# m-dayani/EORB_SLAM

Measured on AMD Instinct MI355X. Metric: front-end frames/s (event-accumulate + extract + match) per GPU; HBM GB/s vs roofline, higher is better.
Workload: dtype f32; 1 GPU; BASELINE.json configs[1]: synthetic 1000000 events/slice on 240x180 (shapes generator, DAVIS sensor pixels; raw (x,y,t,p) records resolved on the GPU through the calibrator's undistortion maps built from the EvETHZ intrinsics, as the reference loader does on the CPU), ev2im_gauss sigma=1 -> ORB-1000 (1.2, 4 levels, FAST 10/0, edge 19) -> SearchForInitialization vs previous slice; input=raw, sequences_per_gpu=1, parallelism=1 GPU

## Files before the change

### eorb_slam_amd/csrc/ev_slots.hip

```cpp
#include "eorb_ctx.h"
#include "ev_common.h"
#include "dev_math.h"
#include "sl_hot_asm.h"
#include <algorithm>
#include <memory>
#include <stdlib.h>
#include <string.h>
#include <vector>

namespace eorb {

constexpr uint32_t kNoSlot = 0xffu;
typedef uint16_t slot_entry;
constexpr uint32_t kEntryTag = 0x1000u;
constexpr int kSlotScatWaves = 8;
constexpr uint16_t kNoGeo = 0xffffu;
constexpr int kCountWaves = 16;

__global__ void sl_assign_kernel(const uint32_t* __restrict__ src_info, int nsrc, int W, int H, int h, int TX,
                                 uint32_t* __restrict__ tile_nslots, uint2* __restrict__ slot_tab, uint16_t* __restrict__ slot_geo,
                                 int* __restrict__ info)
{
    const int i = blockIdx.x * blockDim.x + threadIdx.x;
    if (i >= nsrc) { if (i == nsrc) slot_geo[i] = kNoGeo; return; }
    const uint32_t w = src_info[i];
    const int xi = (int)(int16_t)(w & 0xffff), yi = (int)(int16_t)(w >> 16);
    uint2 o = make_uint2(0u, 0xffffffffu);
    if (xi != -32768) {
        const int x0 = max(xi - h, 0), x1 = min(xi + h, W - 1), y0 = max(yi - h, 0), y1 = min(yi + h, H - 1);
        if (x1 >= x0 && y1 >= y0) {
            const int tx0 = x0 >> 3, tx1 = x1 >> 3, ty0 = y0 >> 3, ty1 = y1 >> 3;
            const int nx = tx1 - tx0 + 1, ny = ty1 - ty0 + 1;
            uint32_t slots = 0xffffffffu;
            for (int dy = 0; dy < ny; dy++)
                for (int dx = 0; dx < nx; dx++) {
                    uint32_t s = atomicAdd(&tile_nslots[(ty0 + dy) * TX + tx0 + dx], 1u);
                    if (s >= kNoSlot) { atomicOr(&info[2], 1); s = 0; }
                    const int sh = 8 * (dy * 2 + dx);
                    slots = (slots & ~(0xffu << sh)) | (s << sh);
                }
            o.x = (uint32_t)tx0 | ((uint32_t)ty0 << 8) | ((uint32_t)nx << 16) | ((uint32_t)ny << 18);
            o.y = slots;
        }
    }
    slot_tab[i] = o;
    slot_geo[i] = o.x ? (uint16_t)((o.x & 0x7f) | (((o.x >> 8) & 0x7f) << 7) | ((((o.x >> 16) & 3) - 1) << 14) | ((((o.x >> 18) & 3) - 1) << 15)) : kNoGeo;
}

__global__ __launch_bounds__(1024) void sl_rowbase_kernel(const uint32_t* __restrict__ nslots, int NT, uint32_t* __restrict__ rowbase,
                                                          int* __restrict__ info)
{
    __shared__ uint32_t wsum[16];
    __shared__ uint32_t wmax[16];
    const int tid = threadIdx.x, lane = tid & 63, wave = tid >> 6;
    const int per = (NT + 1023) / 1024;
    const int t0 = tid * per, t1 = min(t0 + per, NT);
    uint32_t mine = 0, mx = 0;
    for (int t = t0; t < t1; t++) { const uint32_t v = nslots[t]; mine += v; mx = max(mx, v); }
    uint32_t incl = (uint32_t)wave_incl_scan((int)mine);
#pragma unroll
    for (int d = 32; d >= 1; d >>= 1) mx = max(mx, (uint32_t)__shfl_xor((int)mx, d, 64));
    if (lane == 63) wsum[wave] = incl;
    if (lane == 0) wmax[wave] = mx;
    __syncthreads();
    uint32_t before = incl - mine;
    for (int w = 0; w < wave; w++) before += wsum[w];
    for (int t = t0; t < t1; t++) { rowbase[t] = before; before += nslots[t]; }
    if (tid == 1023) {
        uint32_t m = 0;
        for (int w = 0; w < 16; w++) m = max(m, wmax[w]);
// ... 366 lines not shown
        if (tid == NTHR - 1) loff[NT] = (uint16_t)before;
    }
    __syncthreads();
    const uint64_t lt_mask = (lane == 0) ? 0ull : (~0ull >> (64 - lane));
    uint16_t* cw = cntw + wave * NTp;
    const int txr = (TX + R - 1) / R;
    int mbits = 1; while ((1 << mbits) < txr * ((TY + R - 1) / R)) mbits++;
#pragma unroll
    for (int s = 0; s < SMAX; s++) {
        if (s >= S) break;
        const uint32_t rg = rng[s];
        const int tx0 = rg & 0xff, ty0 = (rg >> 8) & 0xff, tx1 = tx0 + (int)((rg >> 16) & 3) - 1, ty1 = ty0 + (int)((rg >> 18) & 3) - 1;
        const bool valid = rg != 0u;
        const uint16_t kloc = (uint16_t)(wave * Q + s * 64 + lane);
#pragma unroll
        for (int cy = 0; cy < R; cy++) {
#pragma unroll
            for (int cx = 0; cx < R; cx++) {
                const int tx = tx0 + ((cx - tx0 % R) + R) % R;
                const int ty = ty0 + ((cy - ty0 % R) + R) % R;
                const bool has = valid && tx <= tx1 && ty <= ty1;
                uint64_t m = __ballot(has);
                if (m == 0ull) continue;
                const int key = has ? ty * TX + tx : 0;
                const int mkey = has ? (ty / R) * txr + (tx / R) : 0;
                for (int b = 0; b < mbits; b++) {
                    const bool bit = (mkey >> b) & 1;
                    const uint64_t bal = __ballot(bit);
                    m &= bit ? bal : ~bal;
                }
                if (has) {
                    const int rank = __popcll(m & lt_mask);
                    const uint32_t base = cw[key];
                    sidx[(uint32_t)loff[key] + base + rank] = (uint16_t)(kloc | ((tx - tx0) << 11) | ((ty - ty0) << 13));
                    if (rank == 0) cw[key] = (uint16_t)(base + (uint32_t)__popcll(m));
                }
            }
        }
    }
    __syncthreads();
    slot_entry* out = entries + (size_t)slice_ebase[cd.slice];
    const int E = loff[NT];
    for (int p = tid; p < E; p += NTHR) {
        const uint32_t sv = sidx[p];
        const int k = sv & 0x7ff;
        const int dx = (sv >> 11) & 3, dy = (sv >> 13) & 3;
        const uint32_t r0 = prng[k];
        const int t = ((int)(r0 >> 8) + dy) * TX + (int)(r0 & 0xff) + dx;
        const uint32_t slot = (pay[k] >> (8 * (dy * 2 + dx))) & 0xffu;
        out[(size_t)gbase[t] + (uint32_t)(p - (int)loff[t])] = (slot_entry)(kEntryTag | slot);
    }
}

template <int stride, int NW >
__global__ __launch_bounds__(64 * NW) void sl_scatter_rank_kernel(const eorb_raw_event* __restrict__ ev, const ChunkDesc* __restrict__ chunks,
                                                                              const uint2* __restrict__ slot_tab, int LW, int LH, int TX, int NT,
                                                                              int chunk_cap, const int64_t* __restrict__ slice_ebase,
                                                                              const uint32_t* __restrict__ segbase, const uint32_t* __restrict__ tile_base,
                                                                              slot_entry* __restrict__ entries)
{
    extern __shared__ unsigned char sm2[];
    __shared__ uint32_t s_wsum[NW];
    constexpr int NTHR = 64 * NW;
    const int tid = threadIdx.x, lane = tid & 63, wave = tid >> 6;
    const int chunk = blockIdx.x;
    const ChunkDesc cd = chunks[chunk];
    const int NTp = (NT + 1) & ~1;
    uint32_t* gbase = (uint32_t*)sm2;
    uint16_t* stile = (uint16_t*)(gbase + NT);
    uint16_t* cntw = stile + (size_t)chunk_cap * 4;
    uint16_t* loff = cntw + NW * NTp;
    uint8_t* sorted = (uint8_t*)(loff + NTp + 2);
    for (int i = tid; i < NW * NTp / 2; i += NTHR) ((uint32_t*)cntw)[i] = 0u;
    const unsigned char* e = (const unsigned char*)ev + (size_t)cd.start * (size_t)(stride < 0 ? -stride : stride);
    const uint32_t xmask = stride == 4 ? 0x7fffu : 0xffffu;
    const bool hashed = stride < 0 || stride == 2;
    const int Q = (((cd.n + NW - 1) / NW) + 63) & ~63;
    const int S = Q >> 6;
    constexpr int SMAX = 4;
    __syncthreads();
    uint32_t* cw32 = (uint32_t*)(cntw + wave * NTp);
    uint32_t rsrc[SMAX];
#pragma unroll
    for (int s = 0; s < SMAX; s++) {
        const int k = wave * Q + s * 64 + lane;
        const uint32_t q = (s < S && k < cd.n) ? sl_load_rec<stride>(e, k) : 0xffffffffu;
        const int x = q == 0xffffffffu ? 0xffff : (int)(q & xmask), y = (int)(q >> 16);
        if (hashed) { const uint32_t row = q & 0x7fffffffu; rsrc[s] = (row != 0x7fffffffu && row < (uint32_t)LW * (uint32_t)LH) ? row : 0xffffffffu; }
        else rsrc[s] = (x < LW && y < LH) ? (uint32_t)y * (uint32_t)LW + x : 0xffffffffu;
    }
    uint2 rst[SMAX];
#pragma unroll
    for (int s = 0; s < SMAX; s++) rst[s] = rsrc[s] != 0xffffffffu ? slot_tab[rsrc[s]] : make_uint2(0u, 0xffffffffu);
    uint32_t rk[SMAX];
#pragma unroll
    for (int s = 0; s < SMAX; s++) {
        const uint32_t rg = rst[s].x;
        const int nx = (rg >> 16) & 3, ny = (rg >> 18) & 3;
        const int tx0 = rg & 0xff, ty0 = (rg >> 8) & 0xff;
        rk[s] = 0u;
#pragma unroll
        for (int j = 0; j < 4; j++) {
#ifdef EORB_TEST_RANK_ORDER_BUG
            const int dx = j & 1, dy = j >> 1;
#else
            const int dx = ((j & 1) - tx0) & 1, dy = ((j >> 1) - ty0) & 1;
#endif
            if (nx && ny && dx < nx && dy < ny) {
                const int t = (ty0 + dy) * TX + tx0 + dx;
                const uint32_t o = atomicAdd(&cw32[t >> 1], 1u << (16 * (t & 1)));
                rk[s] |= ((o >> (16 * (t & 1))) & 0xffu) << (8 * j);
            }
        }
    }
    __syncthreads();
#if defined(EORB_KO_SCAT) && EORB_KO_SCAT == 1
    if (rk[0] == 0x12345678u) entries[0] = 0; return;
#endif
    {
        const int per = (NT + NTHR - 1) / NTHR;
        const int t0 = tid * per, t1 = min(t0 + per, NT);
        uint32_t mine = 0;
        for (int t = t0; t < t1; t++) {
            uint32_t run = 0;
#pragma unroll
            for (int w = 0; w < NW; w++) { const uint32_t v = cntw[w * NTp + t]; cntw[w * NTp + t] = (uint16_t)run; run += v; }
            loff[t] = (uint16_t)run;
            mine += run;
        }
        uint32_t incl = (uint32_t)wave_incl_scan((int)mine);
        if (lane == 63) s_wsum[wave] = incl;
        __syncthreads();
        uint32_t before = incl - mine;
        for (int w = 0; w < wave; w++) before += s_wsum[w];
        for (int t = t0; t < t1; t++) {
            const uint32_t v = loff[t]; loff[t] = (uint16_t)before;
            gbase[t] = tile_base[(size_t)cd.slice * NT + t] + segbase[(size_t)chunk * NT + t] - before;
            before += v;
        }
        if (tid == NTHR - 1) loff[NT] = (uint16_t)before;
    }
    __syncthreads();
#if defined(EORB_KO_SCAT) && EORB_KO_SCAT == 2
    if (rk[0] == 0x12345678u) entries[0] = 0; return;
#endif
    const uint16_t* cw = cntw + wave * NTp;
#pragma unroll
    for (int s = 0; s < SMAX; s++) {
        const uint32_t rg = rst[s].x, sb = rst[s].y;
        const int nx = (rg >> 16) & 3, ny = (rg >> 18) & 3;
        const int tx0 = rg & 0xff, ty0 = (rg >> 8) & 0xff;
#pragma unroll
        for (int j = 0; j < 4; j++) {
#ifdef EORB_TEST_RANK_ORDER_BUG
            const int dx = j & 1, dy = j >> 1;
#else
            const int dx = ((j & 1) - tx0) & 1, dy = ((j >> 1) - ty0) & 1;
#endif
            if (nx && ny && dx < nx && dy < ny) {
                const int t = (ty0 + dy) * TX + tx0 + dx;
                const uint32_t pos = (uint32_t)loff[t] + cw[t] + ((rk[s] >> (8 * j)) & 0xffu);
                sorted[pos] = (uint8_t)((sb >> (8 * (dy * 2 + dx))) & 0xffu);
                stile[pos] = (uint16_t)t;
            }
        }
    }
    __syncthreads();
#if defined(EORB_KO_SCAT) && EORB_KO_SCAT == 3
    if (rk[0] == 0x12345678u) entries[0] = 0; return;
#endif
    slot_entry* out = entries + (size_t)slice_ebase[cd.slice];
    const int E = loff[NT];
    for (int p = tid; p < E; p += NTHR) out[(size_t)(uint32_t)(gbase[stile[p]] + (uint32_t)p)] = (slot_entry)(kEntryTag | sorted[p]);
}

template <int NW>
__global__ __launch_bounds__(64 * NW) void sl_scatter_pre_kernel(const uint64_t* __restrict__ rec, const ChunkDesc* __restrict__ chunks,
                                                                 const uint2* __restrict__ slot_tab, int nsrc, int TX, int NT, int chunk_cap,
                                                                 const int64_t* __restrict__ slice_ebase, const uint16_t* __restrict__ segcnt,
                                                                 const uint32_t* __restrict__ segbase, const uint32_t* __restrict__ tile_base,
                                                                 slot_entry* __restrict__ entries)
{
    extern __shared__ unsigned char sm2[];
    __shared__ uint32_t s_wsum[NW];
    constexpr int NTHR = 64 * NW;
    const int tid = threadIdx.x, lane = tid & 63, wave = tid >> 6;
    const int chunk = blockIdx.x;
    const ChunkDesc cd = chunks[chunk];
    const int NTp = (NT + 1) & ~1;
    uint32_t* gbase = (uint32_t*)sm2;
    uint16_t* stile = (uint16_t*)(gbase + NT);
    uint16_t* loff = stile + (size_t)chunk_cap * 4;
    uint8_t* sorted = (uint8_t*)(loff + NTp + 2);
    const int Q = (((cd.n + NW - 1) / NW) + 63) & ~63;
    const int S = Q >> 6;
    constexpr int SMAX = 4;
    uint64_t rr[SMAX]; uint2 rst[SMAX];
#pragma unroll
    for (int s = 0; s < SMAX; s++) {
        const int k = wave * Q + s * 64 + lane;
        rr[s] = (s < S && k < cd.n) ? rec[cd.start + k] : 0xffffull;
    }
#pragma unroll
    for (int s = 0; s < SMAX; s++) {
        const uint32_t row = (uint32_t)(rr[s] & 0xffffull);
        rst[s] = (row != 0xffffu && row < (uint32_t)nsrc) ? slot_tab[row] : make_uint2(0u, 0xffffffffu);
    }
    {
        const int per = (NT + NTHR - 1) / NTHR;
        const int t0 = tid * per, t1 = min(t0 + per, NT);
        const uint16_t* sc = segcnt + (size_t)chunk * NT;
        uint32_t mine = 0;
        for (int t = t0; t < t1; t++) mine += sc[t];
        uint32_t incl = (uint32_t)wave_incl_scan((int)mine);
        if (lane == 63) s_wsum[wave] = incl;
        __syncthreads();
        uint32_t before = incl - mine;
        for (int w = 0; w < wave; w++) before += s_wsum[w];
        for (int t = t0; t < t1; t++) {
            const uint32_t v = sc[t];
            loff[t] = (uint16_t)before;
            gbase[t] = tile_base[(size_t)cd.slice * NT + t] + segbase[(size_t)chunk * NT + t] - before;
            before += v;
        }
        if (tid == NTHR - 1) loff[NT] = (uint16_t)before;
    }
    __syncthreads();
#if defined(EORB_KO_SCAT) && EORB_KO_SCAT == 2
    if (rst[0].x == 0x12345678u) entries[0] = 0; return;
#endif
#pragma unroll
    for (int s = 0; s < SMAX; s++) {
        const uint32_t rg = rst[s].x, sb = rst[s].y;
        const int nx = (rg >> 16) & 3, ny = (rg >> 18) & 3;
        const int tx0 = rg & 0xff, ty0 = (rg >> 8) & 0xff;
        const uint64_t rk = rr[s] >> 16;
#pragma unroll
        for (int j = 0; j < 4; j++) {
            const int dx = ((j & 1) - tx0) & 1, dy = ((j >> 1) - ty0) & 1;
            if (nx && ny && dx < nx && dy < ny) {
                const int t = (ty0 + dy) * TX + tx0 + dx;
                const uint32_t pos = (uint32_t)loff[t] + (uint32_t)((rk >> (12 * j)) & 0xfffull);
                sorted[pos] = (uint8_t)((sb >> (8 * (dy * 2 + dx))) & 0xffu);
                stile[pos] = (uint16_t)t;
            }
        }
    }
    __syncthreads();
#if defined(EORB_KO_SCAT) && EORB_KO_SCAT == 3
    if (rst[0].x == 0x12345678u) entries[0] = 0; return;
#endif
    slot_entry* out = entries + (size_t)slice_ebase[cd.slice];
    const int E = loff[NT];
    for (int p = tid; p < E; p += NTHR) out[(size_t)(uint32_t)(gbase[stile[p]] + (uint32_t)p)] = (slot_entry)(kEntryTag | sorted[p]);
}

__global__ __launch_bounds__(1024) void sl_rankcheck_kernel(unsigned long long* bad)
{
    __shared__ uint32_t cnt[16 * 64];
    __shared__ uint32_t noise[1024];
    const int lane = threadIdx.x & 63, wave = threadIdx.x >> 6;
    unsigned long long nbad = 0;
    uint32_t h = (uint32_t)(blockIdx.x * 1024 + threadIdx.x) * 2654435761u + 12345u;
    for (int t = 0; t < 64; t++) {
        for (int i = threadIdx.x; i < 16 * 64; i += blockDim.x) cnt[i] = 0;
        __syncthreads();
        h = h * 1664525u + 1013904223u;
        const int spread = 1 << (1 + (t % 7));
        const uint32_t a = ((h >> 9) % spread) + wave * 128;
        const bool act = ((h >> 3) & 7u) != 0u;
        uint32_t r = 0xffffffffu;
        noise[(threadIdx.x * 33 + t) & 1023] = h;
        uint32_t rr[4];
#pragma unroll
        for (int q = 0; q < 4; q++) {
            rr[q] = 0xffffffffu;
            if (act && ((h >> (12 + q)) & 1u)) { const uint32_t o = atomicAdd(&cnt[a >> 1], 1u << (16 * (a & 1))); rr[q] = (o >> (16 * (a & 1))) & 0xffffu; }
        }
#pragma unroll
        for (int q = 0; q < 4; q++) {
            r = rr[q];
            for (int j = 0; j < 64; j++) {
                const uint32_t aj = __shfl(a, j, 64), rj = __shfl(r, j, 64);
                if (r != 0xffffffffu && rj != 0xffffffffu && j < lane && aj == a && !(rj < r)) nbad++;
            }
        }
        __syncthreads();
    }
    if (noise[threadIdx.x] == 0x12345u) nbad += 0;
    if (nbad) atomicAdd(bad, nbad);
}

constexpr int kHotBuckets = 16, kHotCap = 8192;
struct HotDesc { uint32_t slice, tile, cnt, off_lo, off_hi, tx0, ty0, rows_off; };
__global__ __launch_bounds__(256) void sl_plan_kernel(const uint32_t* __restrict__ tile_cnt, const uint32_t* __restrict__ tile_base,
                                                      const int64_t* __restrict__ slice_ebase, int B, int NT, int TX, uint32_t hot_min,
                                                      const uint32_t* __restrict__ nslots, const uint32_t* __restrict__ rowbase,
                                                      uint4* __restrict__ items, uint32_t* __restrict__ tile_w, uint32_t* __restrict__ tile_m,
                                                      uint32_t* __restrict__ ctr, uint32_t* __restrict__ hot_cnt, HotDesc* __restrict__ hot_items,
                                                      uint32_t hot_cap )
{
    extern __shared__ uint32_t pc[];
    __shared__ uint32_t red[8];
    __shared__ uint32_t hb[kHotBuckets], hbase[kHotBuckets];
    uint32_t* hloc = pc + B;
    const int t = blockIdx.x, tid = threadIdx.x;
    const bool hot_ok = hot_min != 0u && nslots[t] <= (uint32_t)SL_HOT_NROWS;
// ... 291 lines not shown
    int* rb = readback_buf(c);
    if (!rb) return set_err(c, EORB_E_HIP, "pinned alloc failed");
    EORB_HIP(c, hipMemcpyAsync(rb + 8, d_info, sizeof(c->sl_hinfo), hipMemcpyDeviceToHost, c->stream));
    c->sl_launched = 1;
    return EORB_OK;
}

int ev_slots_prepare_finish(eorb_ctx* c, int W, int H, int h, int TX, int TY, const float* d_stamps, int stamp_stride, int SWP, float two_sig2, float norm)
{
    if (!c->sl_launched) return EORB_OK;
    c->sl_launched = 0;
    const int nsrc = c->lut_w * c->lut_h, NT = TX * TY;
    memcpy(c->sl_hinfo, readback_buf(c) + 8, sizeof(c->sl_hinfo));
    const int* hinfo = c->sl_hinfo;
    int rc;
    if (c->sl_rank_ok < 0) c->sl_rank_ok = (hinfo[4] == 0 && hinfo[5] == 0) ? 1 : 0;
    if (hinfo[2] || hinfo[1] >= (int)kNoSlot || hinfo[0] <= 0) return EORB_OK;
    if ((rc = ensure(c, c->sl_rows, sizeof(float) * 64 * (size_t)hinfo[0] + 4096 + 256 * 256))) return rc;
    const uint32_t* d_rowbase = (const uint32_t*)c->sl_tile.p + NT;
    sl_rows_kernel<<<(nsrc + 3) / 4, 256, 0, c->stream>>>((const uint32_t*)c->src_info.p, (const uint2*)c->sl_tab.p, nsrc, W, H, h, TX, d_stamps,
                                                            stamp_stride, SWP, (const float2*)c->lut.p, two_sig2, norm, d_rowbase, (float*)c->sl_rows.p);
    EORB_LAUNCH_CHECK(c, "sl_rows_kernel");
    c->sl_null = hinfo[1];
    c->sl_ok = 1;
    return EORB_OK;
}

int ev_slots_prepare(eorb_ctx* c, int W, int H, int h, int TX, int TY, const float* d_stamps, int stamp_stride, int SWP, float two_sig2, float norm)
{
    int rc;
    if (!c->sl_launched) {
        if ((rc = ev_slots_prepare_launch(c, W, H, h, TX, TY))) return rc;
        if (!c->sl_launched) return EORB_OK;
        EORB_HIP(c, hipStreamSynchronize(c->stream));
    }
    return ev_slots_prepare_finish(c, W, H, h, TX, TY, d_stamps, stamp_stride, SWP, two_sig2, norm);
}

static int sl_optin(eorb_ctx* c, int bit, const void* fn, int bytes)
{
    if (c->sl_attr & (1u << bit)) return EORB_OK;
    EORB_HIP(c, hipFuncSetAttribute(fn, hipFuncAttributeMaxDynamicSharedMemorySize, bytes));
    c->sl_attr |= 1u << bit;
    return EORB_OK;
}
static int sl_ncu(eorb_ctx* c)
{
    if (!c->ncu) { hipDeviceProp_t pr; if (hipGetDeviceProperties(&pr, c->device) == hipSuccess) c->ncu = pr.multiProcessorCount; if (c->ncu <= 0) c->ncu = 256; }
    return c->ncu;
}

constexpr int kSlotDeclined = 1;

struct SlotScatterChoice { int chunk, waves; bool rank; size_t lds; };
static size_t sl_lds_rank(int NT, int chunk, int waves) { const int NTp = (NT + 1) & ~1; return ((size_t)NT * 4 + (size_t)chunk * 4 * 2 + (size_t)waves * NTp * 2 + (size_t)(NTp + 2) * 2 + (size_t)chunk * 4 + 15) & ~(size_t)15; }
static size_t sl_lds_pre(int NT, int chunk) { const int NTp = (NT + 1) & ~1; return ((size_t)NT * 4 + (size_t)chunk * 4 * 2 + (size_t)(NTp + 2) * 2 + (size_t)chunk * 4 + 15) & ~(size_t)15; }
static size_t sl_lds_ballot(int NT, int chunk) { const int NTp = (NT + 1) & ~1; return ((size_t)chunk * 4 + (size_t)chunk * 2 + (size_t)chunk * 4 * 2 + (size_t)kSlotScatWaves * NTp * 2 + (size_t)(NTp + 2) * 2 + (size_t)NT * 4 + 15) & ~(size_t)15; }
static bool sl_choose_scatter(const eorb_ctx* c, int NT, int64_t per_slice, bool rank_allowed, SlotScatterChoice* out)
{
    static const int chunk_env = [] { const char* e = getenv("EORB_SLOT_CHUNK"); const int v = e ? atoi(e) : 0; return (v == 256 || v == 1024 || v == 2048 || v == 4096) ? v : 0; }();
    const int pref = chunk_env ? chunk_env : (per_slice >= (int64_t)1 << 18 ? 4096 : (per_slice >= (int64_t)1 << 17 ? 2048 : (per_slice >= (int64_t)1 << 14 ? 1024 : 256)));
    static const int sizes[4] = {4096, 2048, 1024, 256};
    for (int i = 0; i < 4; i++) {
        const int chunk = sizes[i];
        if (chunk > pref) continue;
        if (rank_allowed) {
            const int waves = chunk == 4096 ? 16 : kSlotScatWaves;
            const size_t l = sl_lds_rank(NT, chunk, waves);
            if (l <= (size_t)(chunk == 4096 ? 79 : 158) * 1024) { *out = {chunk, waves, true, l}; return true; }
        }
        if (chunk <= 2048) {
            const size_t l = sl_lds_ballot(NT, chunk);
            if (l <= 64 * 1024) { *out = {chunk, kSlotScatWaves, false, l}; return true; }
        }
    }
    (void)c;
    return false;
}

static int sl_streams(eorb_ctx* c)
{
    if (c->sl_side) return EORB_OK;
    int lo = 0, hi = 0;
    (void)hipDeviceGetStreamPriorityRange(&lo, &hi);
    hipStream_t st[3] = {nullptr, nullptr, nullptr};
    hipEvent_t ev[eorb_ctx::kSlotEvents];
    for (auto& e : ev) e = nullptr;
    bool ok = hipStreamCreateWithPriority(&st[0], hipStreamNonBlocking, hi) == hipSuccess && hipStreamCreateWithFlags(&st[1], hipStreamNonBlocking) == hipSuccess &&
              hipStreamCreateWithFlags(&st[2], hipStreamNonBlocking) == hipSuccess;
    for (int i = 0; ok && i < eorb_ctx::kSlotEvents; i++) ok = hipEventCreateWithFlags(&ev[i], hipEventDisableTiming) == hipSuccess;
    if (!ok) {
        for (auto& e : ev) if (e) (void)hipEventDestroy(e);
        for (auto& q : st) if (q) (void)hipStreamDestroy(q);
        return set_err(c, EORB_E_HIP, "slot form: streams / events");
    }
    c->sl_side = st[0]; c->sl_pstream = st[1]; c->sl_gstream = st[2];
    for (int i = 0; i < eorb_ctx::kSlotEvents; i++) c->sl_ev[i] = ev[i];
    return EORB_OK;
}

static int slots_part(eorb_ctx* c, eorb_ctx::SlotWS& ws, int part, int nparts, const void* d_events, int stride_in, const int64_t* h_offsets, int B,
                      int W, int H, int TX, int TY, float* d_f32, uint32_t* d_minmax_enc, const SlotScatterChoice& sc, const SlotDict* dict)
{
    const int stride = dict ? (dict->rec2 ? 2 : -4) : stride_in;
    const int NT = TX * TY;
    const int64_t nev = h_offsets[B] - h_offsets[0];
    const int chunk = sc.chunk;
    hipStream_t M = c->stream, P = c->sl_pstream, Hs = c->sl_side, G = nparts > 1 ? c->sl_gstream : c->stream;
    hipEvent_t* E = c->sl_ev + 5 * part;
    const bool on_dev = B <= kOffsetsInArg;
    std::vector<ChunkDesc> cds;
    std::vector<int> slice_c0(on_dev ? 0 : B + 1);
    std::vector<int64_t> slice_eb(on_dev ? 0 : B + 1);
    int64_t eb = 0, nch = 0;
    for (int b = 0; b < B; b++) {
        if (!on_dev) slice_c0[b] = (int)nch;
        const int64_t s = h_offsets[b], e = h_offsets[b + 1];
        if (!on_dev) slice_eb[b] = eb;
        eb = (eb + (e - s) * 4 + (int64_t)NT * 16 + 15) & ~(int64_t)15;
        nch += (e - s + chunk - 1) / chunk;
        if (!on_dev)
            for (int64_t k = s; k < e; k += chunk) {
                ChunkDesc cd; cd.start = k; cd.n = (int32_t)std::min<int64_t>(chunk, e - k); cd.slice = b;
                cds.push_back(cd);
            }
    }
// ... 89 lines not shown
            if ((rc = sl_optin(c, 13, (const void*)sl_count_lds_kernel<16, true>, 159 * 1024))) return rc;
            sl_count_lds_kernel<16, true><<<g, 64 * kCountWaves, lds_c, M>>>((const eorb_raw_event*)d_events, d_chunks, nchunks, d_geo, c->lut_w, c->lut_h, TX, NT, d_segcnt, *dict);
            }
        }
        else if (nchunks && cl_env && TX <= 127 && TY <= 127 && lds_c <= 159 * 1024) {
            const uint16_t* d_geo = (const uint16_t*)((const char*)c->sl_tab.p + sizeof(uint2) * nsrc);
            const int g = std::min(ncu, (nchunks + kCountWaves - 1) / kCountWaves);
            static const int tc_env = [] { const char* e = getenv("EORB_SLOT_TRANSCODE"); return e ? atoi(e) : 1; }();
            uint16_t* d_rec16 = nullptr;
            static const int pre_env = [] { const char* e = getenv("EORB_SLOT_PRERANK"); return e ? atoi(e) : 1; }();
            const int pre_on = c->dbg_slot_prerank >= 0 ? c->dbg_slot_prerank : pre_env;
            if (pre_on && (stride == 16 || stride == 4 || stride == 2) && nsrc <= 65535 && sc.rank && sl_lds_pre(NT, chunk) <= 158 * 1024) {
                if ((rc = ensure(c, ws.rec16, sizeof(uint64_t) * (size_t)std::max<int64_t>(h_offsets[B], 1)))) return rc;
                d_rec16 = (uint16_t*)ws.rec16.p;
                prerank = true;
#define SL_COUNTR(ST, BIT) do { if ((rc = sl_optin(c, BIT, (const void*)sl_count_lds_kernel<ST, false, true>, 159 * 1024))) return rc; \
                sl_count_lds_kernel<ST, false, true><<<g, 64 * kCountWaves, lds_c, M>>>(d_ev, d_chunks, nchunks, d_geo, c->lut_w, c->lut_h, TX, NT, d_segcnt, SlotDict{nullptr, 0u, nullptr, nullptr, 0}, d_rec16); } while (0)
                if (stride == 16) SL_COUNTR(16, 18); else if (stride == 4) SL_COUNTR(4, 19); else SL_COUNTR(2, 20);
#undef SL_COUNTR
            }
            else {
            if (tc_env && stride == 16 && nsrc <= 65535 && sc.rank) {
                if ((rc = ensure(c, ws.rec16, sizeof(uint16_t) * (size_t)std::max<int64_t>(h_offsets[B], 1)))) return rc;
                d_rec16 = (uint16_t*)ws.rec16.p;
            }
#define SL_COUNT(ST, BIT) do { if ((rc = sl_optin(c, BIT, (const void*)sl_count_lds_kernel<ST>, 159 * 1024))) return rc; \
                sl_count_lds_kernel<ST><<<g, 64 * kCountWaves, lds_c, M>>>(d_ev, d_chunks, nchunks, d_geo, c->lut_w, c->lut_h, TX, NT, d_segcnt, SlotDict{nullptr, 0u, nullptr, nullptr}, d_rec16); } while (0)
            if (stride == 16) SL_COUNT(16, 0); else if (stride == 4) SL_COUNT(4, 1); else if (stride == 2) SL_COUNT(2, 10); else SL_COUNT(-4, 2);
#undef SL_COUNT
            if (d_rec16) { d_ev = (const eorb_raw_event*)d_rec16; scat_stride = 2; }
            }
        }
        else if (nchunks) {
            if (stride == 16) sl_count_kernel<16><<<nchunks, 256, lds, M>>>(d_ev, d_chunks, d_tab, c->lut_w, c->lut_h, TX, NT, d_segcnt);
            else if (stride == 4) sl_count_kernel<4><<<nchunks, 256, lds, M>>>(d_ev, d_chunks, d_tab, c->lut_w, c->lut_h, TX, NT, d_segcnt);
            else if (stride == 2) sl_count_kernel<2><<<nchunks, 256, lds, M>>>(d_ev, d_chunks, d_tab, c->lut_w, c->lut_h, TX, NT, d_segcnt);
            else sl_count_kernel<-4><<<nchunks, 256, lds, M>>>(d_ev, d_chunks, d_tab, c->lut_w, c->lut_h, TX, NT, d_segcnt);
        }
        ps.reset(); ps.reset(new ProfScope(c, "ev_scan"));
        sl_scan_kernel<<<B, 1024, 0, M>>>(d_slice_c0, d_segcnt, NT, d_segbase, d_tile_cnt, d_tile_base);
        ps.reset();
        EORB_HIP(c, hipEventRecord(E[0], M));
        EORB_HIP(c, hipStreamWaitEvent(P, E[0], 0));
        EORB_HIP(c, hipMemsetAsync(ws.hot.p, 0, 256, P));
        sl_plan_kernel<<<NT, 256, sizeof(uint32_t) * 2 * (size_t)B, P>>>(d_tile_cnt, d_tile_base, d_slice_eb, B, NT, TX, hot_min, d_nslots, d_rowbase,
                                                                               d_items, d_tile_w, d_tile_m, d_ctr, d_hot_cnt, d_hot_items, hot_cap);
        sl_tasks_kernel<<<1, 1024, sizeof(uint32_t) * (size_t)NT, P>>>(d_tile_w, d_tile_m, NT, Gt, max_per_tile, d_scr, d_task, d_hot_cnt, hot_cap);
        EORB_HIP(c, hipEventRecord(E[1], P));
        ProfScope ps2(c, "ev_scatter");
        const int stride = scat_stride;
        if (nchunks && prerank) {
            const size_t lds_p = sl_lds_pre(NT, chunk);
            const uint16_t* d_segcnt_c = d_segcnt;
            if (sc.waves == 16) {
                if ((rc = sl_optin(c, 16, (const void*)sl_scatter_pre_kernel<16>, 159 * 1024))) return rc;
                sl_scatter_pre_kernel<16><<<nchunks, 64 * 16, lds_p, M>>>((const uint64_t*)ws.rec16.p, d_chunks, d_tab, c->lut_w * c->lut_h, TX, NT, chunk, d_slice_eb, d_segcnt_c, d_segbase, d_tile_base, (slot_entry*)ws.entries.p);
            } else {
                if ((rc = sl_optin(c, 17, (const void*)sl_scatter_pre_kernel<8>, 159 * 1024))) return rc;
                sl_scatter_pre_kernel<8><<<nchunks, 64 * 8, lds_p, M>>>((const uint64_t*)ws.rec16.p, d_chunks, d_tab, c->lut_w * c->lut_h, TX, NT, chunk, d_slice_eb, d_segcnt_c, d_segbase, d_tile_base, (slot_entry*)ws.entries.p);
            }
        }
        else if (nchunks && sc.rank) {
#define SL_SCAT(ST, NW, BIT) do { if ((rc = sl_optin(c, BIT, (const void*)sl_scatter_rank_kernel<ST, NW>, 159 * 1024))) return rc; \
                sl_scatter_rank_kernel<ST, NW><<<nchunks, 64 * NW, sc.lds, M>>>(d_ev, d_chunks, d_tab, c->lut_w, c->lut_h, TX, NT, chunk, \
                                                                                   d_slice_eb, d_segbase, d_tile_base, (slot_entry*)ws.entries.p); } while (0)
            if (sc.waves == 16) { if (stride == 16) SL_SCAT(16, 16, 3); else if (stride == 4) SL_SCAT(4, 16, 4); else if (stride == 2) SL_SCAT(2, 16, 11); else SL_SCAT(-4, 16, 5); }
            else { if (stride == 16) SL_SCAT(16, 8, 6); else if (stride == 4) SL_SCAT(4, 8, 7); else if (stride == 2) SL_SCAT(2, 8, 12); else SL_SCAT(-4, 8, 8); }
#undef SL_SCAT
        }
        else if (nchunks)
            sl_scatter_kernel<<<nchunks, 64 * kSlotScatWaves, sc.lds, M>>>(d_ev, d_chunks, d_tab, stride, c->lut_w, c->lut_h, TX, TY, NT, chunk,
                                                                                 d_slice_eb, d_segbase, d_tile_base, (slot_entry*)ws.entries.p);
        EORB_LAUNCH_CHECK(c, "ev_bin (slot) kernels");
    }
    EORB_HIP(c, hipEventRecord(E[2], M));
    {
        SlotGather Pg{d_task, d_items, (const uint8_t*)ws.entries.p, d_nslots, d_rowbase, (const float*)c->sl_rows.p,
                      d_tile_w, d_ctr, d_f32, d_minmax_enc, d_info, (int*)c->status.p, B, W, H, TX, NT, c->sl_null, prio_ref, nullptr};
#ifdef EORB_SLOT_TRACE
        if ((rc = ensure(c, c->sl_trace, sizeof(unsigned long long) * 6 * 16 * (size_t)Gt + 64))) return rc;
        EORB_HIP(c, hipMemsetAsync(c->sl_trace.p, 0, sizeof(unsigned long long) * 6 * 16 * (size_t)Gt + 64, M));
        Pg.trace = (unsigned long long*)c->sl_trace.p + 8;
        c->sl_trace_n = (long long)Gt * 16;
#endif
        if ((rc = sl_optin(c, 9, (const void*)sl_gather_kernel, 160 * 1024))) return rc;
        if (hot_min) {
            static const int hw_env = [] { const char* e = getenv("EORB_SLOT_HOT_WAVES"); return e ? atoi(e) : 0; }();
            const int hw = c->dbg_slot_hot_waves > 0 ? c->dbg_slot_hot_waves : (hw_env > 0 ? hw_env : 8 * ncu);
            EORB_HIP(c, hipStreamWaitEvent(Hs, E[2], 0));
            EORB_HIP(c, hipStreamWaitEvent(Hs, E[1], 0));
            sl_hot_kernel<<<hw, 64, 0, Hs>>>(d_hot_cnt, d_hot_cnt + 32, d_hot_items, kHotCap, (const float*)c->sl_rows.p, (const slot_entry*)ws.entries.p,
                                             d_f32, d_minmax_enc, W, H);
        }
        EORB_HIP(c, hipEventRecord(E[3], Hs));
        if (G != M) EORB_HIP(c, hipStreamWaitEvent(G, E[2], 0));
        EORB_HIP(c, hipStreamWaitEvent(G, E[1], 0));
        {
            ProfScope ps(c, "ev_gather", G);
            sl_gather_kernel<<<Gt, 64 * nw, lds_g, G>>>(Pg);
        }
        EORB_HIP(c, hipEventRecord(E[4], G));
        EORB_LAUNCH_CHECK(c, "sl_gather_kernel");
    }
    return EORB_OK;
}

int ev_slots_accumulate(eorb_ctx* c, const void* d_events, int stride, const int64_t* h_offsets, int B, int W, int H, int TX, int TY,
// ... 43 lines not shown
```

Before: 48650 frames/s.

## Replace per-entry tile index array with run-boundary bitmasks in slot scatter

The scatter kernels no longer store a 16-bit tile id per sorted entry. They record run starts as bits in 64-entry bitmask blocks plus a per-block first-run index, and recover each entry's run with a popcount. gbase is indexed by run rather than tile, and the write-out loop is unrolled by four. The pre-rank kernel also prefetches its first two segment counts and bases, sizes SMAX from the chunk size, and gets its own wave-count choice. This cuts LDS footprint and LDS stores in the sort phase, at the cost of atomicOr marking and popcount work during output.

Result: no change. 49260 frames/s (median of 6 runs) (+1.3%).

```diff
diff --git a/eorb_slam_amd/csrc/ev_slots.hip b/eorb_slam_amd/csrc/ev_slots.hip
--- a/eorb_slam_amd/csrc/ev_slots.hip
+++ b/eorb_slam_amd/csrc/ev_slots.hip
@@ -2,6 +2,7 @@
 #include "ev_common.h"
 #include "dev_math.h"
 #include "sl_hot_asm.h"
+#include "sl_runs.h"
 #include <algorithm>
 #include <memory>
 #include <stdlib.h>
@@ -16,6 +17,9 @@
 constexpr int kSlotScatWaves = 8;
 constexpr uint16_t kNoGeo = 0xffffu;
 constexpr int kCountWaves = 16;
+constexpr int kSlotChunkMax = 4096;
+constexpr int kPreWaves4096 = 16;
+constexpr uint32_t kRunOne = 0x10000u;
 
 __global__ void sl_assign_kernel(const uint32_t* __restrict__ src_info, int nsrc, int W, int H, int h, int TX,
                                  uint32_t* __restrict__ tile_nslots, uint2* __restrict__ slot_tab, uint16_t* __restrict__ slot_geo,
@@ -488,6 +492,27 @@
     }
 }
 
+template <int NTHR>
+__device__ __forceinline__ void sl_runs_out(const uint64_t* marks, const uint16_t* first, const uint32_t* gbase ,
+                                            const uint8_t* sorted, int E, int tid, slot_entry* __restrict__ out)
+{
+    static_assert(NTHR % kRunBlock == 0, "a thread's positions must share their place in the block");
+    constexpr int U = 4;
+    const uint64_t upto = sl_run_upto((uint32_t)tid & (kRunBlock - 1));
+    int p = tid;
+    for (; p + (U - 1) * NTHR < E; p += U * NTHR) {
+        uint32_t r[U], g[U], v[U];
+#pragma unroll
+        for (int u = 0; u < U; u++) { r[u] = sl_run_in_block(marks, first, (uint32_t)(p + u * NTHR) / kRunBlock, upto); v[u] = sorted[p + u * NTHR]; }
+#pragma unroll
+        for (int u = 0; u < U; u++) g[u] = gbase[r[u]];
+#pragma unroll
+        for (int u = 0; u < U; u++) out[(size_t)(uint32_t)(g[u] + (uint32_t)(p + u * NTHR))] = (slot_entry)(kEntryTag | v[u]);
+    }
+    for (; p < E; p += NTHR)
+        out[(size_t)(uint32_t)(gbase[sl_run_in_block(marks, first, (uint32_t)p / kRunBlock, upto)] + (uint32_t)p)] = (slot_entry)(kEntryTag | sorted[p]);
+}
+
 template <int stride, int NW >
 __global__ __launch_bounds__(64 * NW) void sl_scatter_rank_kernel(const eorb_raw_event* __restrict__ ev, const ChunkDesc* __restrict__ chunks,
                                                                               const uint2* __restrict__ slot_tab, int LW, int LH, int TX, int NT,
@@ -502,12 +527,15 @@
     const int chunk = blockIdx.x;
     const ChunkDesc cd = chunks[chunk];
     const int NTp = (NT + 1) & ~1;
-    uint32_t* gbase = (uint32_t*)sm2;
-    uint16_t* stile = (uint16_t*)(gbase + NT);
-    uint16_t* cntw = stile + (size_t)chunk_cap * 4;
-    uint16_t* loff = cntw + NW * NTp;
+    const int NB = sl_run_blocks(chunk_cap * 4);
+    uint64_t* marks = (uint64_t*)sm2;
+    uint32_t* gbase = (uint32_t*)(marks + NB);
+    uint16_t* cntw = (uint16_t*)(gbase + NT);
+    uint16_t* first = cntw + NW * NTp;
+    uint16_t* loff = first + ((NB + 1) & ~1);
     uint8_t* sorted = (uint8_t*)(loff + NTp + 2);
     for (int i = tid; i < NW * NTp / 2; i += NTHR) ((uint32_t*)cntw)[i] = 0u;
+    for (int i = tid; i < NB; i += NTHR) marks[i] = 0ull;
     const unsigned char* e = (const unsigned char*)ev + (size_t)cd.start * (size_t)(stride < 0 ? -stride : stride);
     const uint32_t xmask = stride == 4 ? 0x7fffu : 0xffffu;
     const bool hashed = stride < 0 || stride == 2;
@@ -562,16 +590,21 @@
 #pragma unroll
             for (int w = 0; w < NW; w++) { const uint32_t v = cntw[w * NTp + t]; cntw[w * NTp + t] = (uint16_t)run; run += v; }
             loff[t] = (uint16_t)run;
-            mine += run;
+            mine += run + (run ? kRunOne : 0u);
         }
         uint32_t incl = (uint32_t)wave_incl_scan((int)mine);
         if (lane == 63) s_wsum[wave] = incl;
         __syncthreads();
         uint32_t before = incl - mine;
         for (int w = 0; w < wave; w++) before += s_wsum[w];
+        uint32_t r = before >> 16;
+        before &= 0xffffu;
         for (int t = t0; t < t1; t++) {
             const uint32_t v = loff[t]; loff[t] = (uint16_t)before;
-            gbase[t] = tile_base[(size_t)cd.slice * NT + t] + segbase[(size_t)chunk * NT + t] - before;
+            if (v) {
+                gbase[r] = tile_base[(size_t)cd.slice * NT + t] + segbase[(size_t)chunk * NT + t] - before;
+                sl_run_mark(marks, first, before, before + v, r++);
+            }
             before += v;
         }
         if (tid == NTHR - 1) loff[NT] = (uint16_t)before;
@@ -597,7 +630,6 @@
                 const int t = (ty0 + dy) * TX + tx0 + dx;
                 const uint32_t pos = (uint32_t)loff[t] + cw[t] + ((rk[s] >> (8 * j)) & 0xffu);
                 sorted[pos] = (uint8_t)((sb >> (8 * (dy * 2 + dx))) & 0xffu);
-                stile[pos] = (uint16_t)t;
             }
         }
     }
@@ -605,9 +637,7 @@
 #if defined(EORB_KO_SCAT) && EORB_KO_SCAT == 3
     if (rk[0] == 0x12345678u) entries[0] = 0; return;
 #endif
-    slot_entry* out = entries + (size_t)slice_ebase[cd.slice];
-    const int E = loff[NT];
-    for (int p = tid; p < E; p += NTHR) out[(size_t)(uint32_t)(gbase[stile[p]] + (uint32_t)p)] = (slot_entry)(kEntryTag | sorted[p]);
+    sl_runs_out<NTHR>(marks, first, gbase, sorted, loff[NT], tid, entries + (size_t)slice_ebase[cd.slice]);
 }
 
 template <int NW>
@@ -624,39 +654,55 @@
     const int chunk = blockIdx.x;
     const ChunkDesc cd = chunks[chunk];
     const int NTp = (NT + 1) & ~1;
-    uint32_t* gbase = (uint32_t*)sm2;
-    uint16_t* stile = (uint16_t*)(gbase + NT);
-    uint16_t* loff = stile + (size_t)chunk_cap * 4;
+    const int NB = sl_run_blocks(chunk_cap * 4);
+    uint64_t* marks = (uint64_t*)sm2;
+    uint32_t* gbase = (uint32_t*)(marks + NB);
+    uint16_t* first = (uint16_t*)(gbase + NT);
+    uint16_t* loff = first + ((NB + 1) & ~1);
     uint8_t* sorted = (uint8_t*)(loff + NTp + 2);
+    for (int i = tid; i < NB; i += NTHR) marks[i] = 0ull;
     const int Q = (((cd.n + NW - 1) / NW) + 63) & ~63;
     const int S = Q >> 6;
-    constexpr int SMAX = 4;
+    constexpr int SMAX = kSlotChunkMax / (64 * NW);
     uint64_t rr[SMAX]; uint2 rst[SMAX];
 #pragma unroll
     for (int s = 0; s < SMAX; s++) {
         const int k = wave * Q + s * 64 + lane;
         rr[s] = (s < S && k < cd.n) ? rec[cd.start + k] : 0xffffull;
     }
+    const int per = (NT + NTHR - 1) / NTHR;
+    const int t0 = tid * per, t1 = min(t0 + per, NT);
+    const uint16_t* sc = segcnt + (size_t)chunk * NT;
+    const uint32_t* tbp = tile_base + (size_t)cd.slice * NT;
+    const uint32_t* sbp = segbase + (size_t)chunk * NT;
+    uint32_t c01[2], tb01[2], sb01[2];
+#pragma unroll
+    for (int i = 0; i < 2; i++) {
+        const bool in = t0 + i < t1;
+        c01[i] = in ? sc[t0 + i] : 0u; tb01[i] = in ? tbp[t0 + i] : 0u; sb01[i] = in ? sbp[t0 + i] : 0u;
+    }
 #pragma unroll
     for (int s = 0; s < SMAX; s++) {
         const uint32_t row = (uint32_t)(rr[s] & 0xffffull);
         rst[s] = (row != 0xffffu && row < (uint32_t)nsrc) ? slot_tab[row] : make_uint2(0u, 0xffffffffu);
     }
     {
-        const int per = (NT + NTHR - 1) / NTHR;
-        const int t0 = tid * per, t1 = min(t0 + per, NT);
-        const uint16_t* sc = segcnt + (size_t)chunk * NT;
         uint32_t mine = 0;
-        for (int t = t0; t < t1; t++) mine += sc[t];
+        for (int t = t0; t < t1; t++) { const uint32_t v = t < t0 + 2 ? c01[t - t0] : sc[t]; mine += v + (v ? kRunOne : 0u); }
         uint32_t incl = (uint32_t)wave_incl_scan((int)mine);
         if (lane == 63) s_wsum[wave] = incl;
         __syncthreads();
         uint32_t before = incl - mine;
         for (int w = 0; w < wave; w++) before += s_wsum[w];
+        uint32_t r = before >> 16;
+        before &= 0xffffu;
         for (int t = t0; t < t1; t++) {
-            const uint32_t v = sc[t];
+            const uint32_t v = t < t0 + 2 ? c01[t - t0] : sc[t];
             loff[t] = (uint16_t)before;
-            gbase[t] = tile_base[(size_t)cd.slice * NT + t] + segbase[(size_t)chunk * NT + t] - before;
+            if (v) {
+                gbase[r] = (t < t0 + 2 ? tb01[t - t0] + sb01[t - t0] : tbp[t] + sbp[t]) - before;
+                sl_run_mark(marks, first, before, before + v, r++);
+            }
             before += v;
         }
         if (tid == NTHR - 1) loff[NT] = (uint16_t)before;
@@ -667,6 +713,7 @@
 #endif
 #pragma unroll
     for (int s = 0; s < SMAX; s++) {
+        if (s >= S) break;
         const uint32_t rg = rst[s].x, sb = rst[s].y;
         const int nx = (rg >> 16) & 3, ny = (rg >> 18) & 3;
         const int tx0 = rg & 0xff, ty0 = (rg >> 8) & 0xff;
@@ -678,7 +725,6 @@
                 const int t = (ty0 + dy) * TX + tx0 + dx;
                 const uint32_t pos = (uint32_t)loff[t] + (uint32_t)((rk >> (12 * j)) & 0xfffull);
                 sorted[pos] = (uint8_t)((sb >> (8 * (dy * 2 + dx))) & 0xffu);
-                stile[pos] = (uint16_t)t;
             }
         }
     }
@@ -686,9 +732,7 @@
 #if defined(EORB_KO_SCAT) && EORB_KO_SCAT == 3
     if (rst[0].x == 0x12345678u) entries[0] = 0; return;
 #endif
-    slot_entry* out = entries + (size_t)slice_ebase[cd.slice];
-    const int E = loff[NT];
-    for (int p = tid; p < E; p += NTHR) out[(size_t)(uint32_t)(gbase[stile[p]] + (uint32_t)p)] = (slot_entry)(kEntryTag | sorted[p]);
+    sl_runs_out<NTHR>(marks, first, gbase, sorted, loff[NT], tid, entries + (size_t)slice_ebase[cd.slice]);
 }
 
 __global__ __launch_bounds__(1024) void sl_rankcheck_kernel(unsigned long long* bad)
@@ -1086,26 +1130,29 @@
 
 constexpr int kSlotDeclined = 1;
 
-struct SlotScatterChoice { int chunk, waves; bool rank; size_t lds; };
-static size_t sl_lds_rank(int NT, int chunk, int waves) { const int NTp = (NT + 1) & ~1; return ((size_t)NT * 4 + (size_t)chunk * 4 * 2 + (size_t)waves * NTp * 2 + (size_t)(NTp + 2) * 2 + (size_t)chunk * 4 + 15) & ~(size_t)15; }
-static size_t sl_lds_pre(int NT, int chunk) { const int NTp = (NT + 1) & ~1; return ((size_t)NT * 4 + (size_t)chunk * 4 * 2 + (size_t)(NTp + 2) * 2 + (size_t)chunk * 4 + 15) & ~(size_t)15; }
+struct SlotScatterChoice { int chunk, waves , pre_waves ; bool rank; size_t lds; };
+static size_t sl_lds_runs(int chunk) { const int NB = sl_run_blocks(chunk * 4); return (size_t)NB * 8 + (size_t)((NB + 1) & ~1) * 2; }
+static size_t sl_lds_rank(int NT, int chunk, int waves) { const int NTp = (NT + 1) & ~1; return (sl_lds_runs(chunk) + (size_t)NT * 4 + (size_t)waves * NTp * 2 + (size_t)(NTp + 2) * 2 + (size_t)chunk * 4 + 15) & ~(size_t)15; }
+static size_t sl_lds_pre(int NT, int chunk) { const int NTp = (NT + 1) & ~1; return (sl_lds_runs(chunk) + (size_t)NT * 4 + (size_t)(NTp + 2) * 2 + (size_t)chunk * 4 + 15) & ~(size_t)15; }
 static size_t sl_lds_ballot(int NT, int chunk) { const int NTp = (NT + 1) & ~1; return ((size_t)chunk * 4 + (size_t)chunk * 2 + (size_t)chunk * 4 * 2 + (size_t)kSlotScatWaves * NTp * 2 + (size_t)(NTp + 2) * 2 + (size_t)NT * 4 + 15) & ~(size_t)15; }
 static bool sl_choose_scatter(const eorb_ctx* c, int NT, int64_t per_slice, bool rank_allowed, SlotScatterChoice* out)
 {
     static const int chunk_env = [] { const char* e = getenv("EORB_SLOT_CHUNK"); const int v = e ? atoi(e) : 0; return (v == 256 || v == 1024 || v == 2048 || v == 4096) ? v : 0; }();
     const int pref = chunk_env ? chunk_env : (per_slice >= (int64_t)1 << 18 ? 4096 : (per_slice >= (int64_t)1 << 17 ? 2048 : (per_slice >= (int64_t)1 << 14 ? 1024 : 256)));
+    static const int pw_env = [] { const char* e = getenv("EORB_SLOT_SCAT_WAVES"); const int v = e ? atoi(e) : 0; return (v == 8 || v == 16) ? v : 0; }();
     static const int sizes[4] = {4096, 2048, 1024, 256};
     for (int i = 0; i < 4; i++) {
         const int chunk = sizes[i];
         if (chunk > pref) continue;
+        const int pre_waves = pw_env ? pw_env : (chunk == 4096 ? kPreWaves4096 : kSlotScatWaves);
         if (rank_allowed) {
             const int waves = chunk == 4096 ? 16 : kSlotScatWaves;
             const size_t l = sl_lds_rank(NT, chunk, waves);
-            if (l <= (size_t)(chunk == 4096 ? 79 : 158) * 1024) { *out = {chunk, waves, true, l}; return true; }
+            if (l <= (size_t)(chunk == 4096 ? 79 : 158) * 1024) { *out = {chunk, waves, pre_waves, true, l}; return true; }
         }
         if (chunk <= 2048) {
             const size_t l = sl_lds_ballot(NT, chunk);
-            if (l <= 64 * 1024) { *out = {chunk, kSlotScatWaves, false, l}; return true; }
+            if (l <= 64 * 1024) { *out = {chunk, kSlotScatWaves, pre_waves, false, l}; return true; }
         }
     }
     (void)c;
@@ -1301,7 +1348,7 @@
         if (nchunks && prerank) {
             const size_t lds_p = sl_lds_pre(NT, chunk);
             const uint16_t* d_segcnt_c = d_segcnt;
-            if (sc.waves == 16) {
+            if (sc.pre_waves == 16) {
                 if ((rc = sl_optin(c, 16, (const void*)sl_scatter_pre_kernel<16>, 159 * 1024))) return rc;
                 sl_scatter_pre_kernel<16><<<nchunks, 64 * 16, lds_p, M>>>((const uint64_t*)ws.rec16.p, d_chunks, d_tab, c->lut_w * c->lut_h, TX, NT, chunk, d_slice_eb, d_segcnt_c, d_segbase, d_tile_base, (slot_entry*)ws.entries.p);
             } else {
diff --git a/eorb_slam_amd/csrc/sl_runs.h b/eorb_slam_amd/csrc/sl_runs.h
--- /dev/null
+++ b/eorb_slam_amd/csrc/sl_runs.h
@@ -0,0 +1,55 @@
+#pragma once
+#include <stdint.h>
+
+#if defined(__HIPCC__) || defined(__CUDACC__)
+#define SL_RUNS_HD __host__ __device__ inline
+#else
+#define SL_RUNS_HD inline
+#endif
+
+namespace eorb {
+
+constexpr int kRunBlock = 64;
+
+SL_RUNS_HD int sl_run_blocks(int max_entries) { return (max_entries + kRunBlock - 1) / kRunBlock; }
+
+SL_RUNS_HD void sl_run_mark(uint64_t* marks, uint16_t* first, uint32_t start, uint32_t end, uint32_t r)
+{
+    const uint64_t bit = 1ull << (start & (kRunBlock - 1));
+#if defined(__HIP_DEVICE_COMPILE__)
+    atomicOr((unsigned long long*)&marks[start / kRunBlock], (unsigned long long)bit);
+#else
+    marks[start / kRunBlock] |= bit;
+#endif
+    for (uint32_t b = (start + kRunBlock - 1) / kRunBlock; b * kRunBlock < end; b++) first[b] = (uint16_t)r;
+}
+
+SL_RUNS_HD int sl_run_tables(const uint16_t* loff, int NT, uint64_t* marks, uint16_t* first, uint16_t* run_start)
+{
+    const int nb = sl_run_blocks(loff[NT]);
+    for (int b = 0; b < nb; b++) marks[b] = 0ull;
+    uint32_t r = 0;
+    for (int t = 0; t < NT; t++)
+        if (loff[t + 1] > loff[t]) {
+            if (run_start) run_start[r] = loff[t];
+            sl_run_mark(marks, first, loff[t], loff[t + 1], r);
+            r++;
+        }
+    return (int)r;
+}
+
+SL_RUNS_HD uint64_t sl_run_upto(uint32_t i) { return ((2ull << i) - 1ull) & ~1ull; }
+SL_RUNS_HD uint32_t sl_run_in_block(const uint64_t* marks, const uint16_t* first, uint32_t b, uint64_t upto)
+{
+#if defined(__HIP_DEVICE_COMPILE__)
+    return (uint32_t)first[b] + (uint32_t)__popcll(marks[b] & upto);
+#else
+    return (uint32_t)first[b] + (uint32_t)__builtin_popcountll(marks[b] & upto);
+#endif
+}
+SL_RUNS_HD uint32_t sl_run_of(const uint64_t* marks, const uint16_t* first, uint32_t p)
+{
+    return sl_run_in_block(marks, first, p / kRunBlock, sl_run_upto(p & (kRunBlock - 1)));
+}
+
+}
```
